# htcr/sam_road

Hardware: NVIDIA H100
Metric: 512x512 ViT-B tiles/sec (higher is better)
Workload: dtype f16 operands / f32 accumulate

## Files before the change

sam_road_b200/csrc/common.cu:

```cuda
#include "common.cuh"
#include "ops.h"

#include <atomic>
#include <cstdarg>
#include <cstdio>
#include <map>
#include <mutex>
#include <utility>

namespace srb {

static thread_local char g_last_error[1024] = "";

void set_last_error(const char* fmt, ...) {
  va_list ap;
  va_start(ap, fmt);
  vsnprintf(g_last_error, sizeof(g_last_error), fmt, ap);
  va_end(ap);
}
const char* get_last_error() { return g_last_error; }

static std::atomic<uint64_t> g_launches{0};
static void note_launch() { g_launches.fetch_add(1, std::memory_order_relaxed); }
uint64_t launch_count(bool reset) {
// ... 71 lines not shown
  static int cached[64] = {0};
  int dev = 0;
  if (cudaGetDevice(&dev) != cudaSuccess || dev < 0 || dev >= 64) return 132;
  if (cached[dev] == 0) {
    int n = 0;
    if (cudaDeviceGetAttribute(&n, cudaDevAttrMultiProcessorCount, dev) != cudaSuccess || n <= 0)
      return 132;
    cached[dev] = n;
  }
  return cached[dev];
}

typedef CUresult (*PFN_encodeTiled)(CUtensorMap*, CUtensorMapDataType, cuuint32_t, void*,
                                    const cuuint64_t*, const cuuint64_t*, const cuuint32_t*,
                                    const cuuint32_t*, CUtensorMapInterleave, CUtensorMapSwizzle,
                                    CUtensorMapL2promotion, CUtensorMapFloatOOBfill);

static PFN_encodeTiled get_encode_fn() {
  static PFN_encodeTiled fn = nullptr;
  static std::once_flag once;
  std::call_once(once, [] {
    void* p = nullptr;
    cudaDriverEntryPointQueryResult qres;
    if (cudaGetDriverEntryPoint("cuTensorMapEncodeTiled", &p, cudaEnableDefault, &qres) ==
            cudaSuccess &&
        qres == cudaDriverEntryPointSuccess)
      fn = reinterpret_cast<PFN_encodeTiled>(p);
  });
  return fn;
}

int make_tmap_f16_2d(CUtensorMap* out, const void* base, uint64_t rows, uint64_t cols,
                     uint64_t ld_elems, uint32_t box_rows, uint32_t box_cols) {
  PFN_encodeTiled fn = get_encode_fn();
  SRB_REQUIRE(fn != nullptr, "cuTensorMapEncodeTiled driver entry point not available");
  SRB_REQUIRE((reinterpret_cast<uintptr_t>(base) & 15u) == 0, "TMA base %p not 16-byte aligned",
              base);
  SRB_REQUIRE((ld_elems * 2) % 16 == 0, "TMA row pitch %llu B not a multiple of 16",
              (unsigned long long)(ld_elems * 2));
  cuuint64_t gdim[2] = {cols, rows};
  cuuint64_t gstr[1] = {ld_elems * 2};
  cuuint32_t box[2] = {box_cols, box_rows};
  cuuint32_t estr[2] = {1, 1};
  CUresult r = fn(out, CU_TENSOR_MAP_DATA_TYPE_FLOAT16, 2, const_cast<void*>(base), gdim, gstr, box,
                  estr, CU_TENSOR_MAP_INTERLEAVE_NONE, CU_TENSOR_MAP_SWIZZLE_128B,
                  CU_TENSOR_MAP_L2_PROMOTION_L2_256B, CU_TENSOR_MAP_FLOAT_OOB_FILL_NONE);
  SRB_REQUIRE(r == CUDA_SUCCESS,
              "cuTensorMapEncodeTiled failed (%d) rows=%llu cols=%llu ld=%llu box=%ux%u", (int)r,
              (unsigned long long)rows, (unsigned long long)cols, (unsigned long long)ld_elems,
              box_rows, box_cols);
  return 0;
}

int make_tmap_f16_4d(CUtensorMap* out, const void* base, const uint64_t dims[4],
                     const uint64_t strides_elems[3], const uint32_t box[4]) {
  PFN_encodeTiled fn = get_encode_fn();
  SRB_REQUIRE(fn != nullptr, "cuTensorMapEncodeTiled driver entry point not available");
  SRB_REQUIRE((reinterpret_cast<uintptr_t>(base) & 15u) == 0, "TMA base %p not 16-byte aligned",
              base);
  cuuint64_t gdim[4] = {dims[0], dims[1], dims[2], dims[3]};
  cuuint64_t gstr[3] = {strides_elems[0] * 2, strides_elems[1] * 2, strides_elems[2] * 2};
  for (int i = 0; i < 3; ++i)
    SRB_REQUIRE(gstr[i] % 16 == 0, "TMA stride %d = %llu B not a multiple of 16", i,
                (unsigned long long)gstr[i]);
  cuuint32_t bx[4] = {box[0], box[1], box[2], box[3]};
  cuuint32_t estr[4] = {1, 1, 1, 1};
  CUresult r = fn(out, CU_TENSOR_MAP_DATA_TYPE_FLOAT16, 4, const_cast<void*>(base), gdim, gstr, bx,
                  estr, CU_TENSOR_MAP_INTERLEAVE_NONE, CU_TENSOR_MAP_SWIZZLE_128B,
                  CU_TENSOR_MAP_L2_PROMOTION_L2_256B, CU_TENSOR_MAP_FLOAT_OOB_FILL_NONE);
  SRB_REQUIRE(r == CUDA_SUCCESS, "cuTensorMapEncodeTiled(4D) failed (%d)", (int)r);
  return 0;
}

int make_tmap_f32_4d_dense(CUtensorMap* out, const void* base, const uint64_t dims[4],
                           const uint64_t strides_bytes[3], const uint32_t box[4]) {
  PFN_encodeTiled fn = get_encode_fn();
  SRB_REQUIRE(fn != nullptr, "cuTensorMapEncodeTiled driver entry point not available");
  SRB_REQUIRE((reinterpret_cast<uintptr_t>(base) & 15u) == 0, "TMA base %p not 16-byte aligned",
              base);
  cuuint64_t gdim[4] = {dims[0], dims[1], dims[2], dims[3]};
  cuuint64_t gstr[3] = {strides_bytes[0], strides_bytes[1], strides_bytes[2]};
  for (int i = 0; i < 3; ++i)
    SRB_REQUIRE(gstr[i] % 16 == 0, "TMA stride %d = %llu B not a multiple of 16", i,
                (unsigned long long)gstr[i]);
  cuuint32_t bx[4] = {box[0], box[1], box[2], box[3]};
  cuuint32_t estr[4] = {1, 1, 1, 1};
  CUresult r = fn(out, CU_TENSOR_MAP_DATA_TYPE_FLOAT32, 4, const_cast<void*>(base), gdim, gstr, bx,
                  estr, CU_TENSOR_MAP_INTERLEAVE_NONE, CU_TENSOR_MAP_SWIZZLE_NONE,
                  CU_TENSOR_MAP_L2_PROMOTION_L2_256B, CU_TENSOR_MAP_FLOAT_OOB_FILL_NONE);
  SRB_REQUIRE(r == CUDA_SUCCESS, "cuTensorMapEncodeTiled(4D f32) failed (%d)", (int)r);
  return 0;
}

typedef CUresult (*PFN_streamMemOp32)(CUstream, CUdeviceptr, cuuint32_t, unsigned int);
static PFN_streamMemOp32 get_memop_fn(const char* name) {
  void* p = nullptr;
  cudaDriverEntryPointQueryResult qres;
  if (cudaGetDriverEntryPoint(name, &p, cudaEnableDefault, &qres) == cudaSuccess && qres == cudaDriverEntryPointSuccess)
    return reinterpret_cast<PFN_streamMemOp32>(p);
  return nullptr;
}
int stream_write_value32(void* addr, uint32_t value, cudaStream_t st) {
  static PFN_streamMemOp32 fn = get_memop_fn("cuStreamWriteValue32");
  SRB_REQUIRE(fn != nullptr, "cuStreamWriteValue32 driver entry point not available");
  const CUresult r = fn(reinterpret_cast<CUstream>(st), reinterpret_cast<CUdeviceptr>(addr), value, 0 );
  SRB_REQUIRE(r == CUDA_SUCCESS, "cuStreamWriteValue32 failed (%d)", static_cast<int>(r));
// ... 12 lines not shown
```

sam_road_b200/csrc/common.cuh:

```cuda
#pragma once

#include <cuda.h>
#include <cuda_fp16.h>
#include <cuda_runtime.h>
#include <stdint.h>

namespace srb {

void set_last_error(const char* fmt, ...);

#define SRB_CUDA_OK(expr)                                                                  \
  do {                                                                                     \
    cudaError_t _e = (expr);                                                               \
    if (_e != cudaSuccess) {                                                               \
      ::srb::set_last_error("%s:%d: %s -> %s", __FILE__, __LINE__, #expr,                  \
                            cudaGetErrorString(_e));                                       \
      return 1;                                                                            \
    }                                                                                      \
  } while (0)

#define SRB_REQUIRE(cond, ...)                                                             \
  do {                                                                                     \
    if (!(cond)) {                                                                         \
      ::srb::set_last_error(__VA_ARGS__);                                                  \
// ... 126 lines not shown

__device__ __forceinline__ void mbar_init(uint64_t* bar, uint32_t count) {
  asm volatile("mbarrier.init.shared::cta.b64 [%0], %1;" ::"r"(smem_u32(bar)), "r"(count));
}
__device__ __forceinline__ void fence_barrier_init() {
  asm volatile("fence.mbarrier_init.release.cluster;" ::: "memory");
}
__device__ __forceinline__ void fence_proxy_async_smem() {
  asm volatile("fence.proxy.async.shared::cta;" ::: "memory");
}
__device__ __forceinline__ void mbar_arrive_expect_tx(uint64_t* bar, uint32_t bytes) {
  asm volatile("mbarrier.arrive.expect_tx.shared::cta.b64 _, [%0], %1;" ::"r"(smem_u32(bar)),
               "r"(bytes)
               : "memory");
}
__device__ __forceinline__ void mbar_arrive(uint64_t* bar) {
  asm volatile("mbarrier.arrive.shared::cta.b64 _, [%0];" ::"r"(smem_u32(bar)) : "memory");
}
__device__ __forceinline__ bool mbar_try_wait(uint64_t* bar, uint32_t parity) {
  uint32_t ok;
  asm volatile(
      "{\n\t"
      ".reg .pred P1;\n\t"
      "mbarrier.try_wait.parity.shared::cta.b64 P1, [%1], %2;\n\t"
      "selp.b32 %0, 1, 0, P1;\n\t"
      "}\n"
      : "=r"(ok)
      : "r"(smem_u32(bar)), "r"(parity)
      : "memory");
  return ok != 0;
}
__device__ __forceinline__ void mbar_wait(uint64_t* bar, uint32_t parity) {
  while (!mbar_try_wait(bar, parity)) {
  }
}

__device__ __forceinline__ void tma_prefetch_desc(const CUtensorMap* tm) {
  asm volatile("prefetch.tensormap [%0];" ::"l"(reinterpret_cast<uint64_t>(tm)) : "memory");
}
__device__ __forceinline__ void tma_load_2d(void* smem_dst, const CUtensorMap* tm, uint64_t* bar,
                                            int32_t c0, int32_t c1) {
  asm volatile(
      "cp.async.bulk.tensor.2d.shared::cluster.global.mbarrier::complete_tx::bytes"
      " [%0], [%1, {%3, %4}], [%2];"
      ::"r"(smem_u32(smem_dst)), "l"(reinterpret_cast<uint64_t>(tm)), "r"(smem_u32(bar)),
      "r"(c0), "r"(c1)
      : "memory");
}
__device__ __forceinline__ void tma_store_4d(const CUtensorMap* tm, const void* smem_src, int32_t c0,
                                             int32_t c1, int32_t c2, int32_t c3) {
  asm volatile("cp.async.bulk.tensor.4d.global.shared::cta.bulk_group [%0, {%2, %3, %4, %5}], [%1];"
               ::"l"(reinterpret_cast<uint64_t>(tm)), "r"(smem_u32(smem_src)), "r"(c0), "r"(c1), "r"(c2),
               "r"(c3)
               : "memory");
}
__device__ __forceinline__ void bulk_commit_group() {
  asm volatile("cp.async.bulk.commit_group;" ::: "memory");
}
template <int N>
__device__ __forceinline__ void bulk_wait_group_read() {
  asm volatile("cp.async.bulk.wait_group.read %0;" ::"n"(N) : "memory");
}
template <int N>
__device__ __forceinline__ void bulk_wait_group() {
  asm volatile("cp.async.bulk.wait_group %0;" ::"n"(N) : "memory");
}
__device__ __forceinline__ void tma_load_4d(void* smem_dst, const CUtensorMap* tm, uint64_t* bar,
                                            int32_t c0, int32_t c1, int32_t c2, int32_t c3) {
  asm volatile(
      "cp.async.bulk.tensor.4d.shared::cluster.global.mbarrier::complete_tx::bytes"
      " [%0], [%1, {%3, %4, %5, %6}], [%2];"
      ::"r"(smem_u32(smem_dst)), "l"(reinterpret_cast<uint64_t>(tm)), "r"(smem_u32(bar)),
      "r"(c0), "r"(c1), "r"(c2), "r"(c3)
      : "memory");
}

__device__ __forceinline__ uint64_t wgmma_desc_k128(uint32_t smem_addr) {
  uint64_t d = 0;
  d |= static_cast<uint64_t>((smem_addr >> 4) & 0x3FFFu);
  d |= static_cast<uint64_t>(1) << 16;
  d |= static_cast<uint64_t>(1024u >> 4) << 32;
  d |= static_cast<uint64_t>(1) << 62;
  return d;
}
__device__ __forceinline__ void wgmma_fence() {
  asm volatile("wgmma.fence.sync.aligned;" ::: "memory");
}
__device__ __forceinline__ void wgmma_commit() {
  asm volatile("wgmma.commit_group.sync.aligned;" ::: "memory");
}
template <int N>
__device__ __forceinline__ void wgmma_wait() {
  asm volatile("wgmma.wait_group.sync.aligned %0;" ::"n"(N) : "memory");
}
template <int R>
__device__ __forceinline__ void wgmma_fence_operand(float (&d)[R]) {
#pragma unroll
  for (int i = 0; i < R; ++i) asm volatile("" : "+f"(d[i])::"memory");
}
template <int R>
__device__ __forceinline__ void setmaxnreg_inc() {
  asm volatile("setmaxnreg.inc.sync.aligned.u32 %0;" ::"n"(R));
}
template <int R>
__device__ __forceinline__ void setmaxnreg_dec() {
  asm volatile("setmaxnreg.dec.sync.aligned.u32 %0;" ::"n"(R));
// ... 18 lines not shown
      "}\n"
      : "+f"(d[0]), "+f"(d[1]), "+f"(d[2]), "+f"(d[3]), "+f"(d[4]), "+f"(d[5]), "+f"(d[6]), "+f"(d[7]),
        "+f"(d[8]), "+f"(d[9]), "+f"(d[10]), "+f"(d[11]), "+f"(d[12]), "+f"(d[13]), "+f"(d[14]), "+f"(d[15]),
        "+f"(d[16]), "+f"(d[17]), "+f"(d[18]), "+f"(d[19]), "+f"(d[20]), "+f"(d[21]), "+f"(d[22]), "+f"(d[23]),
        "+f"(d[24]), "+f"(d[25]), "+f"(d[26]), "+f"(d[27]), "+f"(d[28]), "+f"(d[29]), "+f"(d[30]), "+f"(d[31]),
        "+f"(d[32]), "+f"(d[33]), "+f"(d[34]), "+f"(d[35]), "+f"(d[36]), "+f"(d[37]), "+f"(d[38]), "+f"(d[39]),
        "+f"(d[40]), "+f"(d[41]), "+f"(d[42]), "+f"(d[43]), "+f"(d[44]), "+f"(d[45]), "+f"(d[46]), "+f"(d[47]),
        "+f"(d[48]), "+f"(d[49]), "+f"(d[50]), "+f"(d[51]), "+f"(d[52]), "+f"(d[53]), "+f"(d[54]), "+f"(d[55]),
        "+f"(d[56]), "+f"(d[57]), "+f"(d[58]), "+f"(d[59]), "+f"(d[60]), "+f"(d[61]), "+f"(d[62]), "+f"(d[63])
      : "l"(desc_a), "l"(desc_b), "r"(accumulate));
}

__device__ __forceinline__ void wgmma_m64n256k16(float (&d)[128], uint64_t desc_a, uint64_t desc_b,
                                             uint32_t accumulate) {
  asm volatile(
      "{\n\t"
      ".reg .pred p;\n\t"
      "setp.ne.b32 p, %130, 0;\n\t"
      "wgmma.mma_async.sync.aligned.m64n256k16.f32.f16.f16 "
      "{"
      "%0, %1, %2, %3, %4, %5, %6, %7, %8, %9, %10, %11, %12, %13, %14, %15, "
      "%16, %17, %18, %19, %20, %21, %22, %23, %24, %25, %26, %27, %28, %29, %30, %31, "
      "%32, %33, %34, %35, %36, %37, %38, %39, %40, %41, %42, %43, %44, %45, %46, %47, "
      "%48, %49, %50, %51, %52, %53, %54, %55, %56, %57, %58, %59, %60, %61, %62, %63, "
      "%64, %65, %66, %67, %68, %69, %70, %71, %72, %73, %74, %75, %76, %77, %78, %79, "
      "%80, %81, %82, %83, %84, %85, %86, %87, %88, %89, %90, %91, %92, %93, %94, %95, "
      "%96, %97, %98, %99, %100, %101, %102, %103, %104, %105, %106, %107, %108, %109, %110, %111, "
      "%112, %113, %114, %115, %116, %117, %118, %119, %120, %121, %122, %123, %124, %125, %126, %127"
      "}, %128, %129, p, 1, 1, 0, 0;\n\t"
      "}\n"
      : "+f"(d[0]), "+f"(d[1]), "+f"(d[2]), "+f"(d[3]), "+f"(d[4]), "+f"(d[5]), "+f"(d[6]), "+f"(d[7]),
        "+f"(d[8]), "+f"(d[9]), "+f"(d[10]), "+f"(d[11]), "+f"(d[12]), "+f"(d[13]), "+f"(d[14]), "+f"(d[15]),
        "+f"(d[16]), "+f"(d[17]), "+f"(d[18]), "+f"(d[19]), "+f"(d[20]), "+f"(d[21]), "+f"(d[22]), "+f"(d[23]),
        "+f"(d[24]), "+f"(d[25]), "+f"(d[26]), "+f"(d[27]), "+f"(d[28]), "+f"(d[29]), "+f"(d[30]), "+f"(d[31]),
        "+f"(d[32]), "+f"(d[33]), "+f"(d[34]), "+f"(d[35]), "+f"(d[36]), "+f"(d[37]), "+f"(d[38]), "+f"(d[39]),
        "+f"(d[40]), "+f"(d[41]), "+f"(d[42]), "+f"(d[43]), "+f"(d[44]), "+f"(d[45]), "+f"(d[46]), "+f"(d[47]),
        "+f"(d[48]), "+f"(d[49]), "+f"(d[50]), "+f"(d[51]), "+f"(d[52]), "+f"(d[53]), "+f"(d[54]), "+f"(d[55]),
        "+f"(d[56]), "+f"(d[57]), "+f"(d[58]), "+f"(d[59]), "+f"(d[60]), "+f"(d[61]), "+f"(d[62]), "+f"(d[63]),
        "+f"(d[64]), "+f"(d[65]), "+f"(d[66]), "+f"(d[67]), "+f"(d[68]), "+f"(d[69]), "+f"(d[70]), "+f"(d[71]),
        "+f"(d[72]), "+f"(d[73]), "+f"(d[74]), "+f"(d[75]), "+f"(d[76]), "+f"(d[77]), "+f"(d[78]), "+f"(d[79]),
        "+f"(d[80]), "+f"(d[81]), "+f"(d[82]), "+f"(d[83]), "+f"(d[84]), "+f"(d[85]), "+f"(d[86]), "+f"(d[87]),
        "+f"(d[88]), "+f"(d[89]), "+f"(d[90]), "+f"(d[91]), "+f"(d[92]), "+f"(d[93]), "+f"(d[94]), "+f"(d[95]),
        "+f"(d[96]), "+f"(d[97]), "+f"(d[98]), "+f"(d[99]), "+f"(d[100]), "+f"(d[101]), "+f"(d[102]), "+f"(d[103]),
        "+f"(d[104]), "+f"(d[105]), "+f"(d[106]), "+f"(d[107]), "+f"(d[108]), "+f"(d[109]), "+f"(d[110]), "+f"(d[111]),
        "+f"(d[112]), "+f"(d[113]), "+f"(d[114]), "+f"(d[115]), "+f"(d[116]), "+f"(d[117]), "+f"(d[118]), "+f"(d[119]),
        "+f"(d[120]), "+f"(d[121]), "+f"(d[122]), "+f"(d[123]), "+f"(d[124]), "+f"(d[125]), "+f"(d[126]), "+f"(d[127])
      : "l"(desc_a), "l"(desc_b), "r"(accumulate));
}


int make_tmap_f16_2d(CUtensorMap* out, const void* base, uint64_t rows, uint64_t cols,
                     uint64_t ld_elems, uint32_t box_rows, uint32_t box_cols = 64);

int make_tmap_f16_4d(CUtensorMap* out, const void* base, const uint64_t dims[4],
                     const uint64_t strides_elems[3], const uint32_t box[4]);
int make_tmap_f32_4d_dense(CUtensorMap* out, const void* base, const uint64_t dims[4],
                           const uint64_t strides_bytes[3], const uint32_t box[4]);

}
```

sam_road_b200/csrc/gemm_ops.cu:

```cuda
#include <cstring>

#include "gemm_tc.cuh"
#include "ops.h"

namespace srb {


static inline bool use_bn256(int M, int N) {
  if (N % 256 != 0) return false;
  const long tiles256 = static_cast<long>((M + kGemmBM - 1) / kGemmBM) * (N / 256);
  return tiles256 >= device_sm_count();
}

int gemm_f16out(const __half* A, int lda, const __half* W, int ldw, int M, int N, int K,
                const float* bias, int act, __half* out, int ldo, cudaStream_t st) {
  SRB_REQUIRE(act == ACT_NONE || act == ACT_GELU || act == ACT_RELU,
              "gemm_f16out: act=%d must be 0 (none), 1 (GELU) or 2 (ReLU)", act);
  EpiF16::Params p{out, bias, ldo, act};
  SRB_REQUIRE(ldo % 8 == 0, "gemm_f16out: ldo=%d must be a multiple of 8", ldo);
  SRB_REQUIRE(reinterpret_cast<uintptr_t>(out) % 16 == 0, "gemm_f16out: out must be 16-byte aligned");
  return launch_gemm_pp<EpiF16>(A, lda, W, ldw, M, N, K, p, st);
}

int gemm_f32out(const __half* A, int lda, const __half* W, int ldw, int M, int N, int K,
                const float* bias, const float* resid, const float* pos, int pos_rows, float* out,
                int ldo, cudaStream_t st) {
  EpiF32::Params p{out, bias, resid, pos, ldo, pos_rows > 0 ? pos_rows : 1, N};
  SRB_REQUIRE(ldo % 4 == 0, "gemm_f32out: ldo=%d must be a multiple of 4", ldo);
  return launch_gemm_pp<EpiF32>(A, lda, W, ldw, M, N, K, p, st);
}

int gemm_ln(const __half* A, int lda, const __half* W, int ldw, int M, int N, int K,
            const float* bias, const float* resid, const float* gamma, const float* beta, float eps,
            int group, int act, __half* out16, float* out32, float* out_nchw, int tokens, int ldo,
            cudaStream_t st, int conv_s) {
  SRB_REQUIRE(act == ACT_NONE || act == ACT_GELU || act == ACT_RELU,
              "gemm_ln: act=%d must be 0 (none), 1 (GELU) or 2 (ReLU)", act);
  SRB_REQUIRE(group == 64 || group == 128 || group == 256, "gemm_ln: group=%d must be 64, 128 or 256", group);
  SRB_REQUIRE(N % group == 0, "gemm_ln: N=%d not a multiple of group=%d", N, group);
  EpiLN::Params p{out16, out32, out_nchw, bias, resid, gamma, beta, eps, ldo, group, act,
                  tokens > 0 ? tokens : 1, N};
  if (group == 256 || use_bn256(M, N))
    return launch_gemm_tc<256, 3, EpiLN>(A, lda, W, ldw, M, N, K, p, st, conv_s);
  return launch_gemm_tc<128, 5, EpiLN>(A, lda, W, ldw, M, N, K, p, st, conv_s);
}

template <bool kPerToken>
static int launch_dec_final(const __half* A, int lda, const __half* W, int ldw, int M, int K,
                            const float* bias3, const float* w4, const float* bias4, int s, int P,
                            float* scores, float* logits, cudaStream_t st) {
  typename EpiDecFinal<kPerToken>::Params p;
  memset(&p, 0, sizeof(p));
  const int B = M / (16 * s * s);
  const uint64_t rowb = static_cast<uint64_t>(P) * 2 * sizeof(float);
  const uint64_t dims[4] = {static_cast<uint64_t>(P) * 2, 2, 2, static_cast<uint64_t>(B) * P / 4};
  const uint64_t strides[3] = {rowb, 2 * rowb, 4 * rowb};
  const uint32_t box[4] = {kPerToken ? 32u : 64u, 2, 1, 4};
  if (scores) { if (int rc = make_tmap_f32_4d_dense(&p.tm_scores, scores, dims, strides, box)) return rc; }
  if (logits) { if (int rc = make_tmap_f32_4d_dense(&p.tm_logits, logits, dims, strides, box)) return rc; }
  p.has_scores = scores != nullptr;
  p.has_logits = logits != nullptr;
  p.bias3 = bias3; p.w4 = w4; p.bias4 = bias4; p.s = s; p.P = P;
  return launch_gemm_tc<128, 5, EpiDecFinal<kPerToken>>(A, lda, W, ldw, M, 128, K, p, st);
}

int gemm_dec_final(const __half* A, int lda, const __half* W, int ldw, int M, int K,
                   const float* bias3, const float* w4, const float* bias4, int s, int P,
                   float* scores, float* logits, cudaStream_t st) {
  SRB_REQUIRE(P == 16 * s && M % (16 * s * s) == 0, "gemm_dec_final: M=%d s=%d P=%d inconsistent", M, s, P);
  if (s % 2 == 0) return launch_dec_final<false>(A, lda, W, ldw, M, K, bias3, w4, bias4, s, P, scores, logits, st);
  return launch_dec_final<true>(A, lda, W, ldw, M, K, bias3, w4, bias4, s, P, scores, logits, st);
}

__global__ void gemm_ref_simt_kernel(const __half* __restrict__ A, int lda,
                                     const __half* __restrict__ W, int ldw, int M, int N, int K,
                                     float* __restrict__ out, int ldo) {
  const int n = blockIdx.x * blockDim.x + threadIdx.x;
  const int m = blockIdx.y;
  if (n >= N || m >= M) return;
  const __half* a = A + static_cast<size_t>(m) * lda;
  const __half* w = W + static_cast<size_t>(n) * ldw;
// ... 21 lines not shown
```

sam_road_b200/csrc/gemm_tc.cuh:

```cuda
#pragma once

#include "common.cuh"
#include "ops.h"

namespace srb {

constexpr int kGemmBM = 128;
constexpr int kGemmBK = 64;
constexpr int kGemmThreads = 384;
constexpr int kGemmEpiWarps = 8;
constexpr int kGemmScratchFloats = 32 * 36;


struct AccRow {
  const float* p;
  __device__ __forceinline__ void load(int chunk, float (&v)[32]) const {
    const float4* s = reinterpret_cast<const float4*>(p + chunk * 32);
#pragma unroll
    for (int i = 0; i < 8; ++i) {
      const float4 x = s[i];
      v[4 * i] = x.x; v[4 * i + 1] = x.y; v[4 * i + 2] = x.z; v[4 * i + 3] = x.w;
    }
  }
};

struct FragPos {
  int r0;
  int n_tile;
  int c0;
  __device__ __forceinline__ FragPos(int m_tile, int n_tile_, int w, int lane)
      : r0(m_tile + 16 * w + (lane >> 2)), n_tile(n_tile_), c0(n_tile_ + 2 * (lane & 3)) {}
  __device__ __forceinline__ int row(int q) const { return r0 + 64 * (q >> 1) + 8 * (q & 1); }
  __device__ __forceinline__ bool cols_in(int col, int N) const { return n_tile + col < N; }
};


struct EpiF16 {
  struct Params {
    __half* out;
    const float* bias;
    int ldo;
    int act;
  };
  static __device__ __forceinline__ void run(const Params& p, int M, int N, const FragPos& f,
                                             float (&d)[2][64]) {
    float2 b[16];
#pragma unroll
    for (int j = 0; j < 16; ++j) {
      b[j] = make_float2(0.f, 0.f);
      if (p.bias && f.cols_in(32 * (j >> 2), N)) b[j] = __ldg(reinterpret_cast<const float2*>(p.bias + f.c0 + 8 * j));
    }
    const int t = threadIdx.x & 3;
#pragma unroll
    for (int c = 0; c < 4; ++c) {
      if (!f.cols_in(32 * c, N)) continue;
      const int n = f.n_tile + 8 * (4 * c + t);
#pragma unroll
      for (int q = 0; q < 4; ++q) {
        uint32_t x[4];
#pragma unroll
        for (int u = 0; u < 4; ++u) {
          const int j = 4 * c + u;
          float2 v = make_float2(d[q >> 1][4 * j + 2 * (q & 1)], d[q >> 1][4 * j + 2 * (q & 1) + 1]);
          if (p.bias) { v.x += b[j].x; v.y += b[j].y; }
          if (p.act == ACT_GELU) v = gelu_erf_fast2(v);
          else if (p.act == ACT_RELU) v = make_float2(fmaxf(v.x, 0.0f), fmaxf(v.y, 0.0f));
          x[u] = pack_half2(v.x, v.y);
        }
#pragma unroll
        for (int k = 0; k < 4; k += 2) {
          const uint32_t r = __shfl_xor_sync(0xffffffffu, (t & 1) ? x[k] : x[k + 1], 1);
          if (t & 1) x[k] = r; else x[k + 1] = r;
        }
#pragma unroll
        for (int k = 0; k < 2; ++k) {
          const uint32_t r = __shfl_xor_sync(0xffffffffu, (t & 2) ? x[k] : x[k + 2], 2);
          if (t & 2) x[k] = r; else x[k + 2] = r;
        }
        const int m = f.row(q);
        if (m < M) *reinterpret_cast<uint4*>(p.out + static_cast<size_t>(m) * p.ldo + n) = make_uint4(x[0], x[1], x[2], x[3]);
      }
    }
  }
};

struct EpiF32 {
  struct Params {
    float* out;
    const float* bias;
    const float* resid;
    const float* pos;
    int ldo;
    int pos_rows;
    int n_total;
  };
  static __device__ __forceinline__ void load_resid(const Params& p, int M, int N, const FragPos& f, int c,
                                                    float2 (&r)[8]) {
    const bool in_n = f.cols_in(16 * c, N);
#pragma unroll
    for (int i = 0; i < 8; ++i) {
      const int m = f.row(i & 3);
      r[i] = make_float2(0.f, 0.f);
      if (p.resid && in_n && m < M)
        r[i] = *reinterpret_cast<const float2*>(p.resid + static_cast<size_t>(m) * p.ldo + f.c0 + 8 * (2 * c + (i >> 2)));
    }
  }
  static __device__ __forceinline__ void run(const Params& p, int M, int N, const FragPos& f,
                                             float (&d)[2][64]) {
    int pos_row[4];
#pragma unroll
    for (int q = 0; q < 4; ++q) pos_row[q] = p.pos ? f.row(q) % p.pos_rows : 0;
    float2 nxt[8];
    load_resid(p, M, N, f, 0, nxt);
#pragma unroll
    for (int c = 0; c < 8; ++c) {
      float2 cur[8];
#pragma unroll
      for (int i = 0; i < 8; ++i) cur[i] = nxt[i];
      if (c + 1 < 8) load_resid(p, M, N, f, c + 1, nxt);
      if (!f.cols_in(16 * c, N)) continue;
      float2 b[2], e[8];
#pragma unroll
      for (int jj = 0; jj < 2; ++jj) {
        const int n = f.c0 + 8 * (2 * c + jj);
        b[jj] = p.bias ? __ldg(reinterpret_cast<const float2*>(p.bias + n)) : make_float2(0.f, 0.f);
#pragma unroll
        for (int q = 0; q < 4; ++q)
          e[4 * jj + q] = p.pos && f.row(q) < M
                              ? __ldg(reinterpret_cast<const float2*>(p.pos + static_cast<size_t>(pos_row[q]) * p.n_total + n))
                              : make_float2(0.f, 0.f);
      }
#pragma unroll
      for (int jj = 0; jj < 2; ++jj) {
        const int n = f.c0 + 8 * (2 * c + jj);
        const int j = 2 * c + jj;
#pragma unroll
        for (int q = 0; q < 4; ++q) {
          const int m = f.row(q);
          const float2 r = cur[4 * jj + q];
          float2 x = make_float2(d[q >> 1][4 * j + 2 * (q & 1)] + r.x, d[q >> 1][4 * j + 2 * (q & 1) + 1] + r.y);
          if (p.bias) { x.x += b[jj].x; x.y += b[jj].y; }
          if (p.pos) { x.x += e[4 * jj + q].x; x.y += e[4 * jj + q].y; }
          if (m < M) *reinterpret_cast<float2*>(p.out + static_cast<size_t>(m) * p.ldo + n) = x;
        }
      }
    }
  }
};

struct EpiLN {
  struct Params {
    __half* out16;
    float* out32;
    float* out_nchw;
    const float* bias;
    const float* resid;
    const float* gamma;
    const float* beta;
    float eps;
    int ldo;
    int group;
    int act;
    int tokens;
    int n_total;
  };
  static __device__ __forceinline__ void load_x(const Params& p, int m, bool valid, int n0,
                                                int chunk, const AccRow& row, float (&v)[32]) {
    row.load(chunk, v);
    if (p.bias) {
      const float4* b4 = reinterpret_cast<const float4*>(p.bias + n0);
#pragma unroll
      for (int i = 0; i < 8; ++i) {
        const float4 b = __ldg(b4 + i);
        v[4 * i + 0] += b.x; v[4 * i + 1] += b.y; v[4 * i + 2] += b.z; v[4 * i + 3] += b.w;
      }
    }
    if (p.resid && valid) {
      const float4* r4 =
          reinterpret_cast<const float4*>(p.resid + static_cast<size_t>(m) * p.ldo + n0);
#pragma unroll
      for (int i = 0; i < 8; ++i) {
        const float4 b = r4[i];
        v[4 * i + 0] += b.x; v[4 * i + 1] += b.y; v[4 * i + 2] += b.z; v[4 * i + 3] += b.w;
      }
    }
  }
  static __device__ __forceinline__ void run(const Params& p, int m0, int M, int n_base, int n_cols,
                                             const AccRow& row, float* scratch, int lane) {
    const int m = m0 + lane;
    const bool valid = m < M;
    if (n_cols <= 0) return;
    const bool shared = p.group > n_cols;
    const int span = shared ? n_cols : p.group;
    const int cpg = span >> 5;
    const int ngroups = n_cols / span;
    const float inv_g = 1.0f / static_cast<float>(p.group);
    const int half = (n_base / n_cols) & 1;
    const float* partner = scratch + (half ? -4 : 4) * kGemmScratchFloats;
    const int pair_bar = 1 + ((m0 >> 5) & 3);
// ... 294 lines not shown
        for (int j = 0; j < BN / 8; ++j) {
          *reinterpret_cast<float2*>(accs + r0 * SM::kAccPitch + 8 * j + c0) = make_float2(d[4 * j], d[4 * j + 1]);
          *reinterpret_cast<float2*>(accs + (r0 + 8) * SM::kAccPitch + 8 * j + c0) =
              make_float2(d[4 * j + 2], d[4 * j + 3]);
        }
      }
      named_bar_sync(6 + g, 128);
      const int m0 = m_blk * kGemmBM + q * 32;
      const int n_tile = min(BN, N - n_blk * BN);
      const int col0 = half * (BN / 2);
      const int n_cols = max(0, min(BN / 2, n_tile - col0));
      AccRow row{accs + (q * 32 + lane) * SM::kAccPitch + col0};
      Epi::run(ep, m0, M, n_blk * BN + col0, n_cols, row, scratch, lane);
      fence_proxy_async_smem();
      __syncwarp();
      if (lane == 0) mbar_arrive(accfree_bar);
    }
    Epi::drain(lane);
  }
}

template <int BN, int STAGES, class Epi>
int launch_gemm_tc(const __half* A, int lda, const __half* W, int ldw, int M, int N, int K,
                   const typename Epi::Params& ep, cudaStream_t stream, int conv_s = 0) {
  using SM = GemmSmem<BN, STAGES>;
  SRB_REQUIRE(M > 0 && N > 0 && K > 0, "gemm: empty problem M=%d N=%d K=%d", M, N, K);
  SRB_REQUIRE(N % 32 == 0, "gemm: N=%d must be a multiple of 32", N);
  SRB_REQUIRE(K % 8 == 0 && lda % 8 == 0 && ldw % 8 == 0,
              "gemm: K/lda/ldw (%d/%d/%d) must be multiples of 8", K, lda, ldw);
  CUtensorMap tmA, tmB;
  if (conv_s > 0) {
    const int C = lda;
    SRB_REQUIRE(K == 9 * C && C % kGemmBK == 0 && kGemmBM % conv_s == 0 && (conv_s * conv_s) % kGemmBM == 0 &&
                    M % (conv_s * conv_s) == 0,
                "gemm conv3x3: unsupported shape M=%d K=%d C=%d s=%d", M, K, C, conv_s);
    const uint64_t dims[4] = {static_cast<uint64_t>(C), static_cast<uint64_t>(conv_s),
                              static_cast<uint64_t>(conv_s), static_cast<uint64_t>(M / (conv_s * conv_s))};
    const uint64_t strides[3] = {static_cast<uint64_t>(C), static_cast<uint64_t>(conv_s) * C,
                                 static_cast<uint64_t>(conv_s) * conv_s * C};
    const uint32_t box[4] = {kGemmBK, static_cast<uint32_t>(conv_s), static_cast<uint32_t>(kGemmBM / conv_s), 1};
    if (int rc = make_tmap_f16_4d(&tmA, A, dims, strides, box)) return rc;
  } else {
    if (int rc = make_tmap_f16_2d(&tmA, A, M, K, lda, kGemmBM)) return rc;
  }
  if (int rc = make_tmap_f16_2d(&tmB, W, N, K, ldw, BN)) return rc;
  auto kern = gemm_tc_kernel<BN, STAGES, Epi>;
  SRB_TRY(allow_dynamic_smem(kern, SM::kTotal));
  const int num_tiles = ((M + kGemmBM - 1) / kGemmBM) * ((N + BN - 1) / BN);
  const int grid = num_tiles < device_sm_count() ? num_tiles : device_sm_count();
  SRB_LAUNCH(kern, grid, kGemmThreads, SM::kTotal, stream, tmA, tmB, M, N, K, ep, conv_s);
  return 0;
}

enum { TR_ORDER_WAIT, TR_ORDER_DONE, TR_FIRST_FULL, TR_LAST_ISSUE, TR_DRAINED, TR_EPI_DONE, TR_EMPTY_WAIT,
       kGemmTraceEvents = 8 };
#ifdef SRB_GEMM_TRACE
struct GemmTrace {
  long long* buf;
  int ctas, tiles;
};
static __device__ GemmTrace g_gemm_trace;
__device__ __forceinline__ long long* gemm_trace_slot(int i) {
  const GemmTrace t = g_gemm_trace;
  if (t.buf == nullptr || static_cast<int>(blockIdx.x) >= t.ctas || i >= t.tiles) return nullptr;
  return t.buf + (static_cast<size_t>(blockIdx.x) * t.tiles + i) * kGemmTraceEvents;
}
#define GEMM_TRACE(...) __VA_ARGS__
#else
#define GEMM_TRACE(...)
#endif

template <int STAGES>
struct GemmPPSmem {
  static constexpr int kABytes = kGemmBM * kGemmBK * 2;
  static constexpr int kBBytes = 128 * kGemmBK * 2;
  static constexpr int kStageBytes = kABytes + kBBytes;
  static constexpr int kBarOffset = STAGES * kStageBytes;
  static constexpr int kTotal = kBarOffset + 256 + 1024;
};

template <int STAGES, class Epi>
__global__ void __launch_bounds__(kGemmThreads, 1)
gemm_pp_kernel(const __grid_constant__ CUtensorMap tmA, const __grid_constant__ CUtensorMap tmB,
               int M, int N, int K, const __grid_constant__ typename Epi::Params ep) {
  using SM = GemmPPSmem<STAGES>;
  extern __shared__ uint8_t smem_raw[];
  const uint32_t raw_addr = smem_u32(smem_raw);
  uint8_t* smem = smem_raw + ((1024u - (raw_addr & 1023u)) & 1023u);

  uint64_t* full_bar = reinterpret_cast<uint64_t*>(smem + SM::kBarOffset);
  uint64_t* empty_bar = full_bar + STAGES;
  uint64_t* order_bar = empty_bar + STAGES;

  const int warp = threadIdx.x >> 5;
  const int lane = threadIdx.x & 31;
  const int wg = warp >> 2;

  const int num_n = (N + 127) / 128;
  const int num_tiles = ((M + kGemmBM - 1) / kGemmBM) * num_n;
  const int num_k = (K + kGemmBK - 1) / kGemmBK;

  if (warp == 0 && lane == 0) {
    tma_prefetch_desc(&tmA);
    tma_prefetch_desc(&tmB);
    for (int s = 0; s < STAGES; ++s) {
      mbar_init(&full_bar[s], 1);
      mbar_init(&empty_bar[s], 4);
    }
    mbar_init(&order_bar[0], 4);
    mbar_init(&order_bar[1], 4);
    fence_barrier_init();
  }
  __syncthreads();

  if (wg == 0) {
    setmaxnreg_dec<40>();
    if (warp == 0 && lane == 0) {
      int stage = 0;
      uint32_t phase = 0;
      GEMM_TRACE(int ti = 0);
      for (int tile = blockIdx.x; tile < num_tiles; tile += gridDim.x) {
        const int m_blk = tile / num_n, n_blk = tile % num_n;
        GEMM_TRACE(long long stall = 0);
        for (int kb = 0; kb < num_k; ++kb) {
          GEMM_TRACE(const long long t0 = clock64());
          mbar_wait(&empty_bar[stage], phase ^ 1u);
          GEMM_TRACE(stall += clock64() - t0);
          uint8_t* sa = smem + stage * SM::kStageBytes;
          mbar_arrive_expect_tx(&full_bar[stage], SM::kStageBytes);
          tma_load_2d(sa, &tmA, &full_bar[stage], kb * kGemmBK, m_blk * kGemmBM);
          tma_load_2d(sa + SM::kABytes, &tmB, &full_bar[stage], kb * kGemmBK, n_blk * 128);
          if (++stage == STAGES) { stage = 0; phase ^= 1u; }
        }
        GEMM_TRACE(if (long long* t = gemm_trace_slot(ti++)) t[TR_EMPTY_WAIT] = stall);
      }
    }
  } else {
    setmaxnreg_inc<232>();
    const int g = wg - 1;
    const int w = warp & 3;
    uint32_t order_phase = 0;
    int i = g;
    for (int tile = blockIdx.x + g * gridDim.x; tile < num_tiles; tile += 2 * gridDim.x, i += 2) {
      const int m_blk = tile / num_n, n_blk = tile % num_n;
      GEMM_TRACE(long long* tr = w == 0 && lane == 0 ? gemm_trace_slot(i) : nullptr;
                 if (tr) tr[TR_ORDER_WAIT] = clock64());
      if (i > 0) {
        mbar_wait(&order_bar[g], order_phase);
        order_phase ^= 1u;
      }
      GEMM_TRACE(if (tr) tr[TR_ORDER_DONE] = clock64());
      const int pos = i * num_k;
      int stage = pos % STAGES;
      uint32_t phase = static_cast<uint32_t>(pos / STAGES) & 1u;
      float d[2][64];
#pragma unroll
      for (int h = 0; h < 2; ++h)
#pragma unroll
        for (int r = 0; r < 64; ++r) d[h][r] = 0.f;
      int prev = -1;
      for (int kb = 0; kb < num_k; ++kb) {
        mbar_wait(&full_bar[stage], phase);
        GEMM_TRACE(if (tr && kb == 0) tr[TR_FIRST_FULL] = clock64());
        const uint32_t a_addr = smem_u32(smem + stage * SM::kStageBytes);
        const uint64_t adesc0 = wgmma_desc_k128(a_addr);
        const uint64_t adesc1 = wgmma_desc_k128(a_addr + 64 * kGemmBK * 2);
        const uint64_t bdesc = wgmma_desc_k128(a_addr + SM::kABytes);
        wgmma_fence_operand(d[0]);
        wgmma_fence_operand(d[1]);
        wgmma_fence();
#pragma unroll
        for (int k = 0; k < kGemmBK / 16; ++k) {
          const uint32_t acc = (kb | k) != 0 ? 1u : 0u;
          wgmma_m64n128k16(d[0], adesc0 + static_cast<uint64_t>(2 * k), bdesc + static_cast<uint64_t>(2 * k), acc);
          wgmma_m64n128k16(d[1], adesc1 + static_cast<uint64_t>(2 * k), bdesc + static_cast<uint64_t>(2 * k), acc);
        }
        wgmma_commit();
        GEMM_TRACE(if (tr && kb == num_k - 1) tr[TR_LAST_ISSUE] = clock64());
        wgmma_wait<1>();
        wgmma_fence_operand(d[0]);
        wgmma_fence_operand(d[1]);
        if (prev >= 0 && lane == 0) mbar_arrive(&empty_bar[prev]);
        prev = stage;
        if (++stage == STAGES) { stage = 0; phase ^= 1u; }
      }
      if (lane == 0) mbar_arrive(&order_bar[g ^ 1]);
      wgmma_wait<0>();
      wgmma_fence_operand(d[0]);
      wgmma_fence_operand(d[1]);
      GEMM_TRACE(if (tr) tr[TR_DRAINED] = clock64());
      if (lane == 0) mbar_arrive(&empty_bar[prev]);
      Epi::run(ep, M, N, FragPos(m_blk * kGemmBM, n_blk * 128, w, lane), d);
      GEMM_TRACE(if (tr) tr[TR_EPI_DONE] = clock64());
    }
  }
}

template <class Epi>
int launch_gemm_pp(const __half* A, int lda, const __half* W, int ldw, int M, int N, int K,
                   const typename Epi::Params& ep, cudaStream_t stream) {
  constexpr int kStages = 5;
  using SM = GemmPPSmem<kStages>;
  SRB_REQUIRE(M > 0 && N > 0 && K > 0, "gemm: empty problem M=%d N=%d K=%d", M, N, K);
  SRB_REQUIRE(N % 32 == 0, "gemm: N=%d must be a multiple of 32", N);
  SRB_REQUIRE(K % 8 == 0 && lda % 8 == 0 && ldw % 8 == 0,
              "gemm: K/lda/ldw (%d/%d/%d) must be multiples of 8", K, lda, ldw);
  CUtensorMap tmA, tmB;
  if (int rc = make_tmap_f16_2d(&tmA, A, M, K, lda, kGemmBM)) return rc;
  if (int rc = make_tmap_f16_2d(&tmB, W, N, K, ldw, 128)) return rc;
  auto kern = gemm_pp_kernel<kStages, Epi>;
  SRB_TRY(allow_dynamic_smem(kern, SM::kTotal));
  const int num_tiles = ((M + kGemmBM - 1) / kGemmBM) * ((N + 127) / 128);
  const int grid = num_tiles < device_sm_count() ? num_tiles : device_sm_count();
  SRB_LAUNCH(kern, grid, kGemmThreads, SM::kTotal, stream, tmA, tmB, M, N, K, ep);
  return 0;
}

}
```

Measured before the change: 1709.

## Route f32 GEMM epilogue residual loads and output stores through TMA staging

The f32-output GEMM epilogue now prefetches residual slabs into per-warp swizzled shared memory with TMA during the mainloop. It combines them with the accumulators in place and writes results back with 2D TMA bulk stores, replacing scattered float2 global loads and stores. The f16 epilogue is specialised at compile time on bias and activation. This adds shared-memory staging, extra mbarriers and bulk-group waits, and raises shared-memory use per block.

```diff
diff --git a/sam_road_b200/csrc/common.cu b/sam_road_b200/csrc/common.cu
--- a/sam_road_b200/csrc/common.cu
+++ b/sam_road_b200/csrc/common.cu
@@ -147,6 +147,27 @@
   return 0;
 }
 
+int make_tmap_f32_2d(CUtensorMap* out, const void* base, uint64_t rows, uint64_t cols, uint64_t ld_elems,
+                     uint32_t box_rows) {
+  PFN_encodeTiled fn = get_encode_fn();
+  SRB_REQUIRE(fn != nullptr, "cuTensorMapEncodeTiled driver entry point not available");
+  SRB_REQUIRE((reinterpret_cast<uintptr_t>(base) & 15u) == 0, "TMA base %p not 16-byte aligned",
+              base);
+  SRB_REQUIRE((ld_elems * 4) % 16 == 0, "TMA row pitch %llu B not a multiple of 16",
+              (unsigned long long)(ld_elems * 4));
+  cuuint64_t gdim[2] = {cols, rows};
+  cuuint64_t gstr[1] = {ld_elems * 4};
+  cuuint32_t box[2] = {32, box_rows};
+  cuuint32_t estr[2] = {1, 1};
+  CUresult r = fn(out, CU_TENSOR_MAP_DATA_TYPE_FLOAT32, 2, const_cast<void*>(base), gdim, gstr, box,
+                  estr, CU_TENSOR_MAP_INTERLEAVE_NONE, CU_TENSOR_MAP_SWIZZLE_128B,
+                  CU_TENSOR_MAP_L2_PROMOTION_L2_256B, CU_TENSOR_MAP_FLOAT_OOB_FILL_NONE);
+  SRB_REQUIRE(r == CUDA_SUCCESS,
+              "cuTensorMapEncodeTiled(f32) failed (%d) rows=%llu cols=%llu ld=%llu box=%ux32", (int)r,
+              (unsigned long long)rows, (unsigned long long)cols, (unsigned long long)ld_elems, box_rows);
+  return 0;
+}
+
 int make_tmap_f16_4d(CUtensorMap* out, const void* base, const uint64_t dims[4],
                      const uint64_t strides_elems[3], const uint32_t box[4]) {
   PFN_encodeTiled fn = get_encode_fn();
diff --git a/sam_road_b200/csrc/common.cuh b/sam_road_b200/csrc/common.cuh
--- a/sam_road_b200/csrc/common.cuh
+++ b/sam_road_b200/csrc/common.cuh
@@ -202,6 +202,11 @@
   asm volatile("cp.async.bulk.tensor.4d.global.shared::cta.bulk_group [%0, {%2, %3, %4, %5}], [%1];"
                ::"l"(reinterpret_cast<uint64_t>(tm)), "r"(smem_u32(smem_src)), "r"(c0), "r"(c1), "r"(c2),
                "r"(c3)
+               : "memory");
+}
+__device__ __forceinline__ void tma_store_2d(const CUtensorMap* tm, const void* smem_src, int32_t c0, int32_t c1) {
+  asm volatile("cp.async.bulk.tensor.2d.global.shared::cta.bulk_group [%0, {%2, %3}], [%1];"
+               ::"l"(reinterpret_cast<uint64_t>(tm)), "r"(smem_u32(smem_src)), "r"(c0), "r"(c1)
                : "memory");
 }
 __device__ __forceinline__ void bulk_commit_group() {
@@ -326,6 +331,9 @@
 int make_tmap_f16_2d(CUtensorMap* out, const void* base, uint64_t rows, uint64_t cols,
                      uint64_t ld_elems, uint32_t box_rows, uint32_t box_cols = 64);
 
+int make_tmap_f32_2d(CUtensorMap* out, const void* base, uint64_t rows, uint64_t cols, uint64_t ld_elems,
+                     uint32_t box_rows);
+
 int make_tmap_f16_4d(CUtensorMap* out, const void* base, const uint64_t dims[4],
                      const uint64_t strides_elems[3], const uint32_t box[4]);
 int make_tmap_f32_4d_dense(CUtensorMap* out, const void* base, const uint64_t dims[4],
diff --git a/sam_road_b200/csrc/gemm_ops.cu b/sam_road_b200/csrc/gemm_ops.cu
--- a/sam_road_b200/csrc/gemm_ops.cu
+++ b/sam_road_b200/csrc/gemm_ops.cu
@@ -25,8 +25,19 @@
 int gemm_f32out(const __half* A, int lda, const __half* W, int ldw, int M, int N, int K,
                 const float* bias, const float* resid, const float* pos, int pos_rows, float* out,
                 int ldo, cudaStream_t st) {
-  EpiF32::Params p{out, bias, resid, pos, ldo, pos_rows > 0 ? pos_rows : 1, N};
   SRB_REQUIRE(ldo % 4 == 0, "gemm_f32out: ldo=%d must be a multiple of 4", ldo);
+  SRB_REQUIRE(reinterpret_cast<uintptr_t>(out) % 16 == 0 && reinterpret_cast<uintptr_t>(resid) % 16 == 0,
+              "gemm_f32out: out and resid must be 16-byte aligned");
+  SRB_REQUIRE(N <= ldo, "gemm_f32out: N=%d wider than the output row pitch ldo=%d", N, ldo);
+  EpiF32::Params p;
+  memset(&p, 0, sizeof(p));
+  if (int rc = make_tmap_f32_2d(&p.tm_out, out, M, N, ldo, 16)) return rc;
+  if (resid) { if (int rc = make_tmap_f32_2d(&p.tm_resid, resid, M, N, ldo, 16)) return rc; }
+  p.bias = bias;
+  p.resid = resid;
+  p.pos = pos;
+  p.pos_rows = pos_rows > 0 ? pos_rows : 1;
+  p.n_total = N;
   return launch_gemm_pp<EpiF32>(A, lda, W, ldw, M, N, K, p, st);
 }
 
diff --git a/sam_road_b200/csrc/gemm_tc.cuh b/sam_road_b200/csrc/gemm_tc.cuh
--- a/sam_road_b200/csrc/gemm_tc.cuh
+++ b/sam_road_b200/csrc/gemm_tc.cuh
@@ -34,22 +34,70 @@
   __device__ __forceinline__ bool cols_in(int col, int N) const { return n_tile + col < N; }
 };
 
+enum { TR_ORDER_WAIT, TR_ORDER_DONE, TR_FIRST_FULL, TR_LAST_ISSUE, TR_DRAINED, TR_EPI_DONE, TR_EMPTY_WAIT,
+       TR_EPI_LOADED, TR_EPI_STAGED, kGemmTraceEvents = 10 };
+#ifdef SRB_GEMM_TRACE
+struct GemmTrace {
+  long long* buf;
+  int ctas, tiles;
+};
+static __device__ GemmTrace g_gemm_trace;
+__device__ __forceinline__ long long* gemm_trace_slot(int i) {
+  const GemmTrace t = g_gemm_trace;
+  if (t.buf == nullptr || static_cast<int>(blockIdx.x) >= t.ctas || i >= t.tiles) return nullptr;
+  return t.buf + (static_cast<size_t>(blockIdx.x) * t.tiles + i) * kGemmTraceEvents;
+}
+__device__ __forceinline__ void gemm_trace_stamp(long long* tr, int event, float dep) {
+  if (tr == nullptr) return;
+  tr[kGemmTraceEvents - 1] = __float_as_int(dep);
+  long long t;
+  asm volatile("mov.u64 %0, %%clock64;" : "=l"(t)::"memory");
+  tr[event] = t;
+}
+#define GEMM_TRACE(...) __VA_ARGS__
+#else
+#define GEMM_TRACE(...)
+#endif
+#if defined(SRB_GEMM_TRACE) && defined(SRB_GEMM_TRACE_NOSTORE)
+#define GEMM_STORE(...)
+#else
+#define GEMM_STORE(...) __VA_ARGS__
+#endif
+
 
 struct EpiF16 {
+  static constexpr int kStageBytes = 0;
   struct Params {
     __half* out;
     const float* bias;
     int ldo;
     int act;
   };
-  static __device__ __forceinline__ void run(const Params& p, int M, int N, const FragPos& f,
-                                             float (&d)[2][64]) {
+  static __device__ __forceinline__ void prefetch(const Params&, int, int, int, int, uint8_t*, uint64_t*) {}
+  static __device__ __forceinline__ void run(const Params& p, int M, int N, const FragPos& f, float (&d)[2][64],
+                                             uint8_t* , uint64_t* , uint32_t (&)[2], long long* tr) {
     float2 b[16];
 #pragma unroll
     for (int j = 0; j < 16; ++j) {
       b[j] = make_float2(0.f, 0.f);
       if (p.bias && f.cols_in(32 * (j >> 2), N)) b[j] = __ldg(reinterpret_cast<const float2*>(p.bias + f.c0 + 8 * j));
     }
+    GEMM_TRACE(float dep = 0.f; for (int j = 0; j < 16; ++j) dep += b[j].x + b[j].y;
+               gemm_trace_stamp(tr, TR_EPI_LOADED, dep));
+    if (p.bias) {
+      if (p.act == ACT_GELU) tile<true, ACT_GELU>(p, M, N, f, d, b, tr);
+      else if (p.act == ACT_RELU) tile<true, ACT_RELU>(p, M, N, f, d, b, tr);
+      else tile<true, ACT_NONE>(p, M, N, f, d, b, tr);
+    } else {
+      if (p.act == ACT_GELU) tile<false, ACT_GELU>(p, M, N, f, d, b, tr);
+      else if (p.act == ACT_RELU) tile<false, ACT_RELU>(p, M, N, f, d, b, tr);
+      else tile<false, ACT_NONE>(p, M, N, f, d, b, tr);
+    }
+  }
+  template <bool kBias, int kAct>
+  static __device__ __forceinline__ void tile(const Params& p, int M, int N, const FragPos& f, float (&d)[2][64],
+                                              const float2 (&b)[16], long long* tr) {
+    GEMM_TRACE(uint32_t sink = 0);
     const int t = threadIdx.x & 3;
 #pragma unroll
     for (int c = 0; c < 4; ++c) {
@@ -62,9 +110,9 @@
         for (int u = 0; u < 4; ++u) {
           const int j = 4 * c + u;
           float2 v = make_float2(d[q >> 1][4 * j + 2 * (q & 1)], d[q >> 1][4 * j + 2 * (q & 1) + 1]);
-          if (p.bias) { v.x += b[j].x; v.y += b[j].y; }
-          if (p.act == ACT_GELU) v = gelu_erf_fast2(v);
-          else if (p.act == ACT_RELU) v = make_float2(fmaxf(v.x, 0.0f), fmaxf(v.y, 0.0f));
+          if (kBias) { v.x += b[j].x; v.y += b[j].y; }
+          if (kAct == ACT_GELU) v = gelu_erf_fast2(v);
+          else if (kAct == ACT_RELU) v = make_float2(fmaxf(v.x, 0.0f), fmaxf(v.y, 0.0f));
           x[u] = pack_half2(v.x, v.y);
         }
 #pragma unroll
@@ -78,47 +126,65 @@
           if (t & 2) x[k] = r; else x[k + 2] = r;
         }
         const int m = f.row(q);
-        if (m < M) *reinterpret_cast<uint4*>(p.out + static_cast<size_t>(m) * p.ldo + n) = make_uint4(x[0], x[1], x[2], x[3]);
-      }
-    }
-  }
+        GEMM_STORE(if (m < M) *reinterpret_cast<uint4*>(p.out + static_cast<size_t>(m) * p.ldo + n) = make_uint4(x[0], x[1], x[2], x[3]));
+        GEMM_TRACE(sink ^= x[0] ^ x[1] ^ x[2] ^ x[3];
+                   if (c == 3 && q == 3) gemm_trace_stamp(tr, TR_EPI_STAGED, __uint_as_float(sink)));
+      }
+    }
+  }
+  static __device__ __forceinline__ void drain(int ) {}
 };
 
 struct EpiF32 {
+  static constexpr int kStageBytes = 4 * 8192;
   struct Params {
-    float* out;
+    CUtensorMap tm_out;
+    CUtensorMap tm_resid;
     const float* bias;
     const float* resid;
     const float* pos;
-    int ldo;
     int pos_rows;
     int n_total;
   };
-  static __device__ __forceinline__ void load_resid(const Params& p, int M, int N, const FragPos& f, int c,
-                                                    float2 (&r)[8]) {
-    const bool in_n = f.cols_in(16 * c, N);
-#pragma unroll
-    for (int i = 0; i < 8; ++i) {
-      const int m = f.row(i & 3);
-      r[i] = make_float2(0.f, 0.f);
-      if (p.resid && in_n && m < M)
-        r[i] = *reinterpret_cast<const float2*>(p.resid + static_cast<size_t>(m) * p.ldo + f.c0 + 8 * (2 * c + (i >> 2)));
-    }
-  }
-  static __device__ __forceinline__ void run(const Params& p, int M, int N, const FragPos& f,
-                                             float (&d)[2][64]) {
+  static __device__ __forceinline__ void load_slab(const Params& p, int M, int N, int n_tile, int row0, int s,
+                                                   uint8_t* stage, uint64_t* bar) {
+    if (n_tile + 32 * s >= N) return;
+    const int boxes = (row0 < M) + (row0 + 64 < M);
+    mbar_arrive_expect_tx(&bar[s & 1], 2048 * boxes);
+    for (int h = 0; h < boxes; ++h)
+      tma_load_2d(stage + 4096 * (s & 1) + 2048 * h, &p.tm_resid, &bar[s & 1], n_tile + 32 * s, row0 + 64 * h);
+  }
+  static __device__ __forceinline__ void prefetch(const Params& p, int M, int N, int n_tile, int row0, uint8_t* stage,
+                                                  uint64_t* bar) {
+    if (p.resid == nullptr) return;
+    bulk_wait_group_read<0>();
+    load_slab(p, M, N, n_tile, row0, 0, stage, bar);
+    load_slab(p, M, N, n_tile, row0, 1, stage, bar);
+  }
+  static __device__ __forceinline__ void run(const Params& p, int M, int N, const FragPos& f, float (&d)[2][64],
+                                             uint8_t* stage, uint64_t* bar, uint32_t (&bar_phase)[2], long long* tr) {
+    const int lane = threadIdx.x & 31;
+    const int row0 = f.r0 - (lane >> 2);
     int pos_row[4];
 #pragma unroll
     for (int q = 0; q < 4; ++q) pos_row[q] = p.pos ? f.row(q) % p.pos_rows : 0;
-    float2 nxt[8];
-    load_resid(p, M, N, f, 0, nxt);
 #pragma unroll
     for (int c = 0; c < 8; ++c) {
-      float2 cur[8];
-#pragma unroll
-      for (int i = 0; i < 8; ++i) cur[i] = nxt[i];
-      if (c + 1 < 8) load_resid(p, M, N, f, c + 1, nxt);
       if (!f.cols_in(16 * c, N)) continue;
+      float* slab = reinterpret_cast<float*>(stage + 4096 * ((c >> 1) & 1));
+      if ((c & 1) == 0) {
+        if (p.resid) {
+          mbar_wait(&bar[(c >> 1) & 1], bar_phase[(c >> 1) & 1]);
+          bar_phase[(c >> 1) & 1] ^= 1u;
+        } else {
+          if (lane == 0) {
+            if (c == 0) bulk_wait_group_read<0>();
+            else bulk_wait_group_read<1>();
+          }
+          __syncwarp();
+        }
+        GEMM_TRACE(if (c == 0) gemm_trace_stamp(tr, TR_EPI_LOADED, slab[0]));
+      }
       float2 b[2], e[8];
 #pragma unroll
       for (int jj = 0; jj < 2; ++jj) {
@@ -132,19 +198,39 @@
       }
 #pragma unroll
       for (int jj = 0; jj < 2; ++jj) {
-        const int n = f.c0 + 8 * (2 * c + jj);
         const int j = 2 * c + jj;
+        const int k = 4 * (c & 1) + 2 * jj + ((lane & 3) >> 1);
 #pragma unroll
         for (int q = 0; q < 4; ++q) {
-          const int m = f.row(q);
-          const float2 r = cur[4 * jj + q];
+          const int row = (lane >> 2) + 8 * (q & 1);
+          float2* at = reinterpret_cast<float2*>(slab + 512 * (q >> 1) + 32 * row + 4 * (k ^ (row & 7)) + 2 * (lane & 1));
+          const float2 r = p.resid ? *at : make_float2(0.f, 0.f);
           float2 x = make_float2(d[q >> 1][4 * j + 2 * (q & 1)] + r.x, d[q >> 1][4 * j + 2 * (q & 1) + 1] + r.y);
           if (p.bias) { x.x += b[jj].x; x.y += b[jj].y; }
           if (p.pos) { x.x += e[4 * jj + q].x; x.y += e[4 * jj + q].y; }
-          if (m < M) *reinterpret_cast<float2*>(p.out + static_cast<size_t>(m) * p.ldo + n) = x;
-        }
-      }
-    }
+          *at = x;
+        }
+      }
+      if (c & 1) {
+        fence_proxy_async_smem();
+        __syncwarp();
+        GEMM_TRACE(if (c == 7) gemm_trace_stamp(tr, TR_EPI_STAGED, 0.f));
+        if (lane == 0) {
+#pragma unroll
+          for (int h = 0; h < 2; ++h)
+            if (row0 + 64 * h < M)
+              GEMM_STORE(tma_store_2d(&p.tm_out, slab + 512 * h, f.n_tile + 32 * (c >> 1), row0 + 64 * h));
+          bulk_commit_group();
+          if (c < 4 && p.resid) {
+            bulk_wait_group_read<0>();
+            load_slab(p, M, N, f.n_tile, row0, (c >> 1) + 2, stage, bar);
+          }
+        }
+      }
+    }
+  }
+  static __device__ __forceinline__ void drain(int lane) {
+    if (lane == 0) bulk_wait_group<0>();
   }
 };
 
@@ -545,38 +631,23 @@
   return 0;
 }
 
-enum { TR_ORDER_WAIT, TR_ORDER_DONE, TR_FIRST_FULL, TR_LAST_ISSUE, TR_DRAINED, TR_EPI_DONE, TR_EMPTY_WAIT,
-       kGemmTraceEvents = 8 };
-#ifdef SRB_GEMM_TRACE
-struct GemmTrace {
-  long long* buf;
-  int ctas, tiles;
-};
-static __device__ GemmTrace g_gemm_trace;
-__device__ __forceinline__ long long* gemm_trace_slot(int i) {
-  const GemmTrace t = g_gemm_trace;
-  if (t.buf == nullptr || static_cast<int>(blockIdx.x) >= t.ctas || i >= t.tiles) return nullptr;
-  return t.buf + (static_cast<size_t>(blockIdx.x) * t.tiles + i) * kGemmTraceEvents;
-}
-#define GEMM_TRACE(...) __VA_ARGS__
-#else
-#define GEMM_TRACE(...)
-#endif
-
-template <int STAGES>
+template <int STAGES, int kEpiBytes>
 struct GemmPPSmem {
   static constexpr int kABytes = kGemmBM * kGemmBK * 2;
   static constexpr int kBBytes = 128 * kGemmBK * 2;
   static constexpr int kStageBytes = kABytes + kBBytes;
-  static constexpr int kBarOffset = STAGES * kStageBytes;
+  static constexpr int kEpiOffset = STAGES * kStageBytes;
+  static constexpr int kBarOffset = kEpiOffset + 2 * kEpiBytes;
   static constexpr int kTotal = kBarOffset + 256 + 1024;
+  static_assert(kTotal <= 227 * 1024, "gemm_pp_kernel: shared memory over the 227 KB an H100 block may use");
+  static_assert((2 * STAGES + 2 + 16) * 8 <= 256, "gemm_pp_kernel: barriers (full, empty, order, staging) over 256 B");
 };
 
 template <int STAGES, class Epi>
 __global__ void __launch_bounds__(kGemmThreads, 1)
 gemm_pp_kernel(const __grid_constant__ CUtensorMap tmA, const __grid_constant__ CUtensorMap tmB,
                int M, int N, int K, const __grid_constant__ typename Epi::Params ep) {
-  using SM = GemmPPSmem<STAGES>;
+  using SM = GemmPPSmem<STAGES, Epi::kStageBytes>;
   extern __shared__ uint8_t smem_raw[];
   const uint32_t raw_addr = smem_u32(smem_raw);
   uint8_t* smem = smem_raw + ((1024u - (raw_addr & 1023u)) & 1023u);
@@ -584,6 +655,7 @@
   uint64_t* full_bar = reinterpret_cast<uint64_t*>(smem + SM::kBarOffset);
   uint64_t* empty_bar = full_bar + STAGES;
   uint64_t* order_bar = empty_bar + STAGES;
+  uint64_t* stage_bar = order_bar + 2;
 
   const int warp = threadIdx.x >> 5;
   const int lane = threadIdx.x & 31;
@@ -602,6 +674,8 @@
     }
     mbar_init(&order_bar[0], 4);
     mbar_init(&order_bar[1], 4);
+    if (Epi::kStageBytes > 0)
+      for (int i = 0; i < 16; ++i) mbar_init(&stage_bar[i], 1);
     fence_barrier_init();
   }
   __syncthreads();
@@ -632,11 +706,14 @@
     setmaxnreg_inc<232>();
     const int g = wg - 1;
     const int w = warp & 3;
-    uint32_t order_phase = 0;
+    uint8_t* staging = smem + SM::kEpiOffset + g * Epi::kStageBytes + w * (Epi::kStageBytes / 4);
+    uint64_t* bar = stage_bar + 2 * (4 * g + w);
+    uint32_t order_phase = 0, bar_phase[2] = {0u, 0u};
     int i = g;
     for (int tile = blockIdx.x + g * gridDim.x; tile < num_tiles; tile += 2 * gridDim.x, i += 2) {
       const int m_blk = tile / num_n, n_blk = tile % num_n;
-      GEMM_TRACE(long long* tr = w == 0 && lane == 0 ? gemm_trace_slot(i) : nullptr;
+      long long* tr = nullptr;
+      GEMM_TRACE(if (w == 0 && lane == 0) tr = gemm_trace_slot(i);
                  if (tr) tr[TR_ORDER_WAIT] = clock64());
       if (i > 0) {
         mbar_wait(&order_bar[g], order_phase);
@@ -670,6 +747,7 @@
         }
         wgmma_commit();
         GEMM_TRACE(if (tr && kb == num_k - 1) tr[TR_LAST_ISSUE] = clock64());
+        if (kb == 0 && lane == 0) Epi::prefetch(ep, M, N, n_blk * 128, m_blk * kGemmBM + 16 * w, staging, bar);
         wgmma_wait<1>();
         wgmma_fence_operand(d[0]);
         wgmma_fence_operand(d[1]);
@@ -683,9 +761,10 @@
       wgmma_fence_operand(d[1]);
       GEMM_TRACE(if (tr) tr[TR_DRAINED] = clock64());
       if (lane == 0) mbar_arrive(&empty_bar[prev]);
-      Epi::run(ep, M, N, FragPos(m_blk * kGemmBM, n_blk * 128, w, lane), d);
+      Epi::run(ep, M, N, FragPos(m_blk * kGemmBM, n_blk * 128, w, lane), d, staging, bar, bar_phase, tr);
       GEMM_TRACE(if (tr) tr[TR_EPI_DONE] = clock64());
     }
+    Epi::drain(lane);
   }
 }
 
@@ -693,7 +772,7 @@
 int launch_gemm_pp(const __half* A, int lda, const __half* W, int ldw, int M, int N, int K,
                    const typename Epi::Params& ep, cudaStream_t stream) {
   constexpr int kStages = 5;
-  using SM = GemmPPSmem<kStages>;
+  using SM = GemmPPSmem<kStages, Epi::kStageBytes>;
   SRB_REQUIRE(M > 0 && N > 0 && K > 0, "gemm: empty problem M=%d N=%d K=%d", M, N, K);
   SRB_REQUIRE(N % 32 == 0, "gemm: N=%d must be a multiple of 32", N);
   SRB_REQUIRE(K % 8 == 0 && lda % 8 == 0 && ldw % 8 == 0,
```

Result: faster. 1767 (median of 6 runs) (+3.4%).
